# indygreg/python-zstandard

Hardware: AMD Instinct MI355X
Metric: GB/s uncompressed throughput, batch decompress of 128 KiB level-3 frames (the decompress half of BASELINE.json's metric; the compress half on the same inputs is this line's 'compress' object) (higher is better)
Workload: dtype u8

## Files before the change

### python-zstandard_amd/csrc/zhip_decode_pipeline.hpp

```cpp
#pragma once
#include "zhip_decode_kernel.hpp"

ZH_DEV void zp_pack_fse(ZdLDS& L, uint32_t* T, uint32_t llLog, uint32_t ofLog, uint32_t mlLog)
{
    const uint32_t lane = zh_lane();
    for (uint32_t u = lane; u < ZP_FSE_CELLS / 2; u += 64) {
        const uint32_t lg = u < 256 ? llLog : u < 512 ? mlLog : ofLog;
        const uint32_t local = (2 * u) & (u < 512 ? 511u : 255u);
        uint32_t pair = 0;
        for (uint32_t k = 0; k < 2; k++) {
            uint32_t cell = 0;
            if (local + k < (1u << lg)) {
                const uint32_t e = L.fse[2 * u + k];
                cell = ((e >> 19) << 10) | (((e & 1023) + (1u << lg)) >> ((e >> 10) & 15));
            }
            pair |= cell << (16 * k);
        }
        T[u] = pair;
    }
}

struct ZpHdr { uint32_t pos, blockMax, hasChecksum, skippable; uint64_t fcs; };
ZH_DEV int zp_frame_header(const ZhipPipeArgs& a, const uint8_t* src, uint32_t srcSize, ZpHdr& h)
{
// ... 934 lines not shown
            uint32_t r[ZP_FSE_CELLS / 128];
#pragma unroll
            for (uint32_t q = 0; q < ZP_FSE_CELLS / 128; q++) r[q] = src[lane + 64 * q];
#pragma unroll
            for (uint32_t q = 0; q < ZP_FSE_CELLS / 128; q++) dstw[lane + 64 * q] = r[q];
        }
        static_assert(ZQ_FRAMES <= 15, "the ring's last column is where the lanes without a frame write");
        uint32_t* const col = L.ring + (active ? slot : 15u);
        const bool idle = isSpare || !active;
        const uint16_t* const Tm = idle ? (const uint16_t*)&L.spare : (const uint16_t*)(L.tab + (size_t)slot * ZP_K2_STRIDE) + tabOff;
        ZdMeta* const m = a.meta + (active ? i : 0u);
        const uint32_t fi = active ? (MB ? a.itemFrame[i] : i) : 0u;
        const uint32_t f = a.first + fi;
        uint32_t nbSeq = 0, logs = 0;
        int32_t pos = 0, pb = -(1 << 30), fin = 0;
        const uint8_t* p0 = (const uint8_t*)a.counters;
        bool ok = active;
        ZpVec16 v0, v1; v0.a = v0.b = v0.c = v0.d = 0; v1 = v0;
        int32_t tb = 0;
        if (active) {
            const uint8_t* src = a.src + a.srcSegs[2 * (size_t)f];
            const uint8_t* p = src + m->seqOff; const uint8_t* end = src + m->seqEnd;
            const uint32_t size = (uint32_t)(end - p);
            logs = m->logs;
            const uint32_t lastB = size ? p[size - 1] : 0u;
            if (lastB == 0) ok = false;
            else {
                nbSeq = m->nbSeq;
                const uint32_t mis = (uint32_t)((uintptr_t)p & 15);
                p0 = p - mis; fin = (int32_t)(8 * mis);
                const int32_t topByte = (int32_t)(mis + size) - 1;
                tb = topByte & ~15;
                v0 = zq_fetch(p0, tb - 16 * (int32_t)role); v1 = zq_fetch(p0, tb - 16 * (int32_t)(role + 4));
                pb = tb - 128;
                pos = 8 * topByte + zh_highbit32(lastB);
            }
        }
        if (ok) { zq_commit(col, tb - 16 * (int32_t)role, v0); zq_commit(col, tb - 16 * (int32_t)(role + 4), v1); }
        zh_sync();
        const uint32_t llLog = logs & 255, ofLog = (logs >> 8) & 255, mlLog = (logs >> 16) & 255;
        const uint32_t myLog = idle ? 9u : role == 0 ? ofLog : role == 1 ? mlLog : llLog;
        const uint32_t kk = 31 - myLog, size = 1u << myLog;
        const uint16_t* const Tb = Tm - size;
        uint32_t state;
        {   const uint32_t initOff = role == 0 ? llLog : role == 1 ? llLog + ofLog : 0u;
            state = idle ? size : size + zq_field(col, pos - (int32_t)(initOff + myLog), myLog);
            pos -= (int32_t)(llLog + ofLog + mlLog); }
        const uint32_t nTrips = zh_first(zh_wave_max(nbSeq)) + 5;
        uint32_t rep0 = 1, rep1 = 4, rep2 = 8;
        if (a.dictEntropy) { rep0 = a.dictEntropy->rep[0]; rep1 = a.dictEntropy->rep[1]; rep2 = a.dictEntropy->rep[2]; }
        if (MB && active && a.frameRecs[fi].firstItem != i) { rep0 = ZP_SYM_REP(0); rep1 = ZP_SYM_REP(1); rep2 = ZP_SYM_REP(2); }
        uint32_t fin0 = rep0, fin1 = rep1, fin2 = rep2;
        rep0 = zh_opaque(rep0); rep1 = zh_opaque(rep1); rep2 = zh_opaque(rep2);
        ZpVec16* outp;
        {
            const uint32_t per = ((nTrips - 5 + 3) & ~3u) + 8;
            const uint32_t nAct = (uint32_t)zh_popc64(zh_ballot(active)) >> 2;
            const uint32_t need16 = per * nAct / 2;
            const uint32_t room16 = zh_first(zh_atomic_add(a.counters + 7, lane == 0 ? need16 : 0u));
            const uint32_t room = room16 * 2;
            if ((uint64_t)room16 + need16 + a.counters[8] > a.arenaBudget16) {
                if (active && isOF) { m->path = 2; if (!MB) { const uint32_t q = zh_atomic_add(a.fallbackCount, 1u); a.fallbackList[q] = f; } }
                zh_sync();
                continue;
            }
            const uint32_t start = room + slot * per + 4;
            if (active && isOF) a.bases[2 * (size_t)i] = start;
            outp = (ZpVec16*)(a.seqArena + (isOF && active ? (size_t)start - 4 : (size_t)room + per - 4));
        }
        const uint32_t outStep = isOF && active ? 2u : 0u;
        uint32_t g1lo = 0, g1hi = 0, g2lo = 0, g2hi = 0, g3lo = 0, g3hi = 0;
        ZpVec16 w0, w1; w0.a = w0.b = w0.c = w0.d = 0; w1 = w0;
        int32_t boff = tb - 16 * (int32_t)role, posEnd = pos; ZpVec16 blk = v0;
        uint32_t pe0 = 0, pe1 = 0, pqE = 0, pbits = 0, pbase = 1;
        for (uint32_t n0 = 0; n0 < nTrips; n0 += 4) {
            zh_sync();
            zq_commit_all(col, boff, blk);
            {   const int32_t t = pb + 128 - (((pos >> 5) << 2) + 4);
                boff = pb - 16 * (int32_t)role + ((int32_t)(role * 16) <= t ? 0 : 128);
                blk = zq_fetch(p0, boff);
                int32_t cnt = (t >> 4) + 1; cnt = cnt < 0 ? 0 : cnt > 4 ? 4 : cnt;
                pb -= 16 * cnt; }
#pragma unroll
            for (uint32_t u = 0; u < 4; u++) {
                const uint32_t n = n0 + u;
                const uint32_t cell = Tb[state];
                ZQ_F1();
                const uint32_t val = pbase + zh_bfe(zh_alignbit(pe1, pe0, pqE), 0, pbits);
                const uint32_t mlv = zh_quad<1>(val), llv = zh_quad<2>(val);
                const uint32_t idx = val - (llv < 1u ? llv : 1u);
                const uint32_t vm3 = val - 3;
                const uint32_t newOff = vm3 < ZP_OF_LIMIT ? vm3 : ZP_OF_LIMIT;
                const uint32_t c3 = val > 3 ? newOff : rep0 - 1;
                const bool i0 = idx == 0, i2 = idx == 2, le1 = idx <= 1;
                const uint32_t a01 = i0 ? rep0 : rep1, b23 = i2 ? rep2 : c3;
                const uint32_t offset = le1 ? a01 : b23;
                ZQ_F2();
                const uint32_t sym = cell >> 10, x = cell & 1023;
                const uint32_t inf = info[sym];
                const uint32_t nb = (uint32_t)__builtin_clz(x) - kk;
                ZQ_F2();
                rep2 = le1 ? rep2 : rep1; rep1 = i0 ? rep1 : rep0; rep0 = offset;
                if (MB) {
                    const bool wasLast = n == nbSeq;
                    fin0 = wasLast ? rep0 : fin0; fin1 = wasLast ? rep1 : fin1; fin2 = wasLast ? rep2 : fin2;
                }
                {   const uint32_t plo = llv | (mlv << 17), phi = (mlv >> 15) | (offset << 3);
                    if (u == 0) {
                        w0.a = g1lo; w0.b = g1hi; w0.c = g2lo; w0.d = g2hi; w1.a = g3lo; w1.b = g3hi; w1.c = plo; w1.d = phi;
#if defined(ZQ_DIAG_NOSTORE)
                        outp += outStep;
#elif defined(ZQ_NT_STORE)
                        {   typedef uint32_t zq_v4 __attribute__((ext_vector_type(4)));
                            zq_v4 t0 = { w0.a, w0.b, w0.c, w0.d }, t1 = { w1.a, w1.b, w1.c, w1.d };
                            __builtin_nontemporal_store(t0, (zq_v4*)outp); __builtin_nontemporal_store(t1, (zq_v4*)(outp + 1)); outp += outStep; }
#else
                        outp[0] = w0; outp[1] = w1; outp += outStep;
#endif
                    } else if (u == 1) { g1lo = plo; g1hi = phi; } else if (u == 2) { g2lo = plo; g2hi = phi; } else { g3lo = plo; g3hi = phi; } }
                ZQ_F2();
                const uint32_t bits = isOF ? sym : inf >> 24;
                const uint32_t P = zh_quad_add<0xCF>(zh_quad_add<0xD3>(bits, bits), bits);
                const uint32_t R = zh_quad_add<0xFE>(zh_quad_add<0xF9>(nb, nb), nb);
                const uint32_t totE = zh_quad<2>(P), totN = zh_quad<0>(R);
                const int32_t pE = pos - (int32_t)totE;
                const int32_t qS = pE - (int32_t)R, qE = pos - (int32_t)P;
                const uint32_t* const wS = (const uint32_t*)((const uint8_t*)col + (zh_bfe((uint32_t)qS, 5, 5) << 6));
                const uint32_t* const wE = (const uint32_t*)((const uint8_t*)col + (zh_bfe((uint32_t)qE, 5, 5) << 6));
                const uint32_t s0 = wS[0], s1 = wS[16];
                pe0 = wE[0]; pe1 = wE[16];
                ZQ_F2();
                pqE = (uint32_t)qE; pbits = bits;
                posEnd = n + 1 == nbSeq ? pE : posEnd;
                pos = pE - (int32_t)totN;
                pbase = isOF ? 1u << (sym & 31) : inf & 0xFFFFFFu;
                ZQ_F2();
                state = (x << nb) + zh_bfe(zh_alignbit(s1, s0, (uint32_t)qS), 0, nb);
                state = zh_pin(state);
            }
            ZH_KEEP4(w0.a, w0.b, w0.c, w0.d); ZH_KEEP4(w1.a, w1.b, w1.c, w1.d);
        }
        if (active && isOF) {
            const int err = !ok ? ZE_CORRUPTION : posEnd != fin ? ZE_CORRUPTION : 0;
            if (err) { m->status = err; m->path = 0; if (!MB) { a.status[f] = err; a.outSizes[f] = 0; } }
            if (MB) { uint32_t* r = a.itemReps + 4 * (size_t)i; r[0] = fin0; r[1] = fin1; r[2] = fin2; }
        }
        zh_sync();
    }
}

#ifndef ZP_ASM_BYTES
#define ZP_ASM_BYTES ZD_ASM_BYTES
#endif
struct ZpExecLDS {
    uint8_t asmb[ZP_ASM_BYTES + 64]; uint16_t mBeg[64]; uint16_t mEnd[64]; uint32_t misc[8];
#if defined(ZP_K3_DIAG_FLOOR) && defined(ZP_FLOOR_LDSPAD)
    uint8_t floorPad[ZP_FLOOR_LDSPAD];
#endif
    uint16_t uEnd[64], uLit[64], dstL[64], dstM[64], lenL[64], lenM[64]; uint32_t srcL[64], srcM[64];
};

ZH_DEV void zp_ld32_lds(const uint8_t* q, uint32_t len, uint64_t r[4])
{
    r[0] = zh_ld64(q); r[1] = zh_ld64(q + 8); r[2] = zh_ld64(q + 16);
    r[3] = zh_ld64(q + (len >= 8 ? len - 8 : 0u));
}

#ifndef ZP_LIT_SHORT
#define ZP_LIT_SHORT 16
#endif
#ifndef ZP_FAR_SHORT
#define ZP_FAR_SHORT 16
#endif
#ifndef ZP_K3_NT
#define ZP_K3_NT 0
#endif
#if ZP_K3_NT & 1
#define ZP_SEQ_LD(p) zh_ldq_nt(p)
#define ZP_LIT_LD64(p) zh_ld64_nt(p)
#else
#define ZP_SEQ_LD(p) (*(p))
#define ZP_LIT_LD64(p) zh_ld64(p)
#endif
#if ZP_K3_NT & 2
#define ZP_FAR_LD64(p) zh_ld64_nt(p)
#else
#define ZP_FAR_LD64(p) zh_ld64(p)
#endif
#define ZD_TP(P, i) do { if (PROF) ZD_T(P, i); } while (0)
ZH_DEV uint32_t zp_sym_resolve(uint32_t v, uint32_t R0, uint32_t R1, uint32_t R2)
{
    if (v <= ZP_OF_LIMIT) return v;
    if (v > ZP_SYM_TOP) return 0xFFFFFFFFu;
    const uint32_t k = (v - (ZP_OF_LIMIT + 1)) >> 23;
    const uint32_t d = ZP_SYM_REP(k) - v;
    const uint32_t r = k == 0 ? R0 : k == 1 ? R1 : R2;
    return r > d ? r - d : 0xFFFFFFFFu;
}

#define ZP_BSYNC() zh_sync()
#ifndef ZP_HIST_KEEP
#define ZP_HIST_KEEP ((ZP_ASM_BYTES * 5u / 16u) & ~15u)
#define ZP_HIST_SLIDE (2u * ZP_HIST_KEEP + 16u)
#endif
static_assert((ZP_HIST_SLIDE >= 2 * ZP_HIST_KEEP + 16 || ZP_HIST_KEEP == 0) && ZP_HIST_KEEP % 16 == 0 && ZP_HIST_SLIDE < ZP_ASM_BYTES, "the slide's source and destination must not overlap");
#ifndef ZP_K3_LITCOPIES
#define ZP_K3_LITCOPIES 3
#endif
enum { ZP_LM_ANY = 0, ZP_LM_ARENA = 1, ZP_LM_RAW = 2, ZP_LM_RLE = 3 };
template <bool DICT, bool PROF, bool MB, int LM>
ZH_DEVFN int zp_exec_block(const ZhipPipeArgs& a, ZpExecLDS& L, const ZdMeta& m, uint32_t t, const uint8_t* src, uint8_t* dst, uint32_t cap, uint64_t cap64,
                           uint32_t blockMax, uint32_t& opRef, uint32_t R0, uint32_t R1, uint32_t R2, ZdProf& P)
{
    const uint32_t lane = zh_lane();
    const uint64_t* seqs = a.seqArena + a.bases[2 * (size_t)t];
    const bool litRLE = LM == ZP_LM_ANY ? m.litMode == 2 : LM == ZP_LM_RLE;
    const bool litRaw = LM == ZP_LM_ANY ? m.litMode == 0 : LM == ZP_LM_RAW;
    const uint32_t rleByte = m.litOff;
    const uint8_t* litPtr = litRaw ? src + m.litOff : a.litArena + (size_t)a.bases[2 * (size_t)t + 1] * 16;
    const uint8_t* const dictEnd = DICT ? a.dictContent + a.dictContentSize : dst;
    const uint32_t dictSize = DICT ? a.dictContentSize : 0u;
    uint32_t hOff = 0;
    uint8_t* asmb = L.asmb;
    const uint32_t blockStart = MB ? opRef : 0u;
    uint32_t op = blockStart, lp = 0, done = 0;
    uint32_t carry = 0;
    const uint32_t nbSeq = m.nbSeq;
    uint64_t qNext = lane < nbSeq ? ZP_SEQ_LD(seqs + lane) : 0;
    const uint32_t lane0 = lane;
    while (done < nbSeq) {
        const uint32_t avail = nbSeq - done < 64 ? nbSeq - done : 64;
        uint32_t myLL = 0, myML = 0, myOF = 1;
        if (lane < avail) { const uint64_t q = qNext; myLL = ZP_SEQ_LL(q); myML = ZP_SEQ_ML(q); myOF = ZP_SEQ_OF(q); if (MB) myOF = zp_sym_resolve(myOF, R0, R1, R2); }
        if (MB && zh_ballot(lane < avail && myOF == ZP_OF_LIMIT)) return ZP_RC_FALLBACK;
        uint32_t incL = zh_scan_add(myLL), incT = zh_scan_add(myLL + myML);
        const uint64_t fits = zh_ballot(lane < avail && incT + carry <= ZP_ASM_BYTES - hOff);
        uint32_t cnt = (uint32_t)zh_popc64(fits);
        const bool big = cnt == 0;
        if (big) cnt = 1;
        qNext = done + cnt + lane < nbSeq ? ZP_SEQ_LD(seqs + done + cnt + lane) : 0;
        const bool act = lane < cnt;
        if (!act) { myLL = 0; myML = 0; myOF = 1; }
        const uint32_t totL = zh_bcast(incL, cnt - 1), totT = zh_bcast(incT, cnt - 1);
        if (lp + totL > m.litSize) return ZE_CORRUPTION;
        if ((uint64_t)op + totT > cap) return ZE_DST_TOO_SMALL;
        if (op + totT - blockStart > blockMax) return ZE_CORRUPTION;
        const uint32_t litStart = lp + incL - myLL;
        const uint32_t ob = op - carry;
        const uint32_t oRel = incT - (myLL + myML) + carry, mRel = oRel + myLL;
        if (zh_ballot(act && myOF - 1 >= ob + mRel + dictSize)) return ZE_CORRUPTION;
        if (big) {
            if (lane < carry) dst[ob + lane] = asmb[lane];
            carry = 0;
            zd_fence();
            const uint32_t bll = zh_bcast(myLL, 0), bml = zh_bcast(myML, 0), bof = zh_bcast(myOF, 0);
            if (litRLE) zd_fill_wave(dst + op, rleByte, bll); else zd_copy_wave(dst + op, litPtr + lp, bll);
            zd_fence();
            zd_match_wave(dst, dictEnd, op + bll, bof, bml);
            zd_fence();
            op += totT; lp += totL; done += 1;
            hOff = 0; asmb = L.asmb;
            continue;
        }
        ZD_TP(P, ZP_STAGE);
        const int32_t sAbs = (int32_t)(ob + mRel) - (int32_t)myOF;
        const bool hasM = act && myML > 0;
        const bool farM = hasM && sAbs + (int32_t)myML <= (int32_t)ob;
        uint32_t nearSkip = 0;
        {
            uint64_t rl[4], rm[4];
            const bool shortL = act && myLL > 0 && myLL <= ZP_LIT_SHORT;
            const bool arenaLit = !litRaw;
            if (arenaLit && !litRLE) {
                const uint8_t* q = litPtr + (shortL ? litStart : 0u);
                rl[0] = ZP_LIT_LD64(q); rl[3] = ZP_LIT_LD64(q + (shortL && myLL >= 8 ? myLL - 8 : 0u));
                if (ZP_LIT_SHORT > 16) { rl[1] = ZP_LIT_LD64(q + 8); rl[2] = ZP_LIT_LD64(q + 16); } else { rl[1] = 0; rl[2] = 0; }
            } else
            if (shortL && !litRLE) zd_ld32(litPtr + litStart, myLL, rl);
            const bool pre = hasM && !farM && sAbs < (int32_t)ob;
            const uint32_t preLen = pre ? (uint32_t)((int32_t)ob - sAbs) : 0u;
            nearSkip = preLen;
            const uint32_t lenMi = farM ? myML : preLen;
            const bool strad = DICT && (farM || pre) && sAbs < 0 && sAbs + (int32_t)lenMi > 0;
            const uint8_t* const mSrc = !DICT || sAbs >= 0 ? dst + sAbs : dictEnd + sAbs;
            const bool shortM = (farM || pre) && lenMi <= ZP_FAR_SHORT && !strad;
            const bool inH = (farM || pre) && sAbs >= (int32_t)(ob - hOff);
            if (!zh_ballot(shortM && !inH && sAbs >= 0 && (uint64_t)sAbs + 32 > cap64) && cap64 >= 32) {
                const uint8_t* q = shortM && !inH ? mSrc : dst;
                rm[0] = ZP_FAR_LD64(q); rm[3] = ZP_FAR_LD64(q + (shortM && lenMi >= 8 ? lenMi - 8 : 0u));
                if (ZP_FAR_SHORT > 16) { rm[1] = ZP_FAR_LD64(q + 8); rm[2] = ZP_FAR_LD64(q + 16); } else { rm[1] = 0; rm[2] = 0; }
            } else
            if (shortM && !inH) zd_ld32(mSrc, lenMi, rm);
            if (shortM && inH) { const uint8_t* hq = asmb + (sAbs - (int32_t)ob); rm[0] = zh_ld64(hq); rm[1] = 0; rm[2] = 0; rm[3] = zh_ld64(hq + (lenMi >= 8 ? lenMi - 8 : 0u)); }
            const bool longL = act && myLL > ZP_LIT_SHORT && !litRLE, longM = (farM || pre) && !shortM && !strad;
            const uint32_t uL = longL ? (myLL + 15) >> 4 : 0u, uM = longM ? (lenMi + 15) >> 4 : 0u;
            const uint32_t ue = zh_scan_add(uL + uM);
            const uint32_t U = zh_bcast(ue, 63);
            zh_v16 uv; uv.lo = 0; uv.hi = 0; uint8_t* udp = asmb;
            if (U) {
                L.uEnd[lane] = (uint16_t)ue; L.uLit[lane] = (uint16_t)uL;
                L.srcL[lane] = litStart; L.dstL[lane] = (uint16_t)oRel; L.lenL[lane] = (uint16_t)myLL;
                L.srcM[lane] = (uint32_t)sAbs; L.dstM[lane] = (uint16_t)mRel; L.lenM[lane] = (uint16_t)lenMi;
                ZP_BSYNC();
#define ZP_UNIT(u) do { uint32_t j_ = 0; for (uint32_t stp_ = 32; stp_; stp_ >>= 1) if (L.uEnd[j_ + stp_ - 1] <= (u)) j_ += stp_; \
                    uint32_t k_ = (u) - (j_ ? (uint32_t)L.uEnd[j_ - 1] : 0u); const uint32_t nl_ = L.uLit[j_]; const bool isL_ = k_ < nl_; if (!isL_) k_ -= nl_; \
                    const uint32_t len_ = isL_ ? L.lenL[j_] : L.lenM[j_]; const uint32_t off_ = 16 * k_ + 16 <= len_ ? 16 * k_ : len_ - 16; \
                    const int32_t sm_ = (int32_t)L.srcM[j_]; \
                    if (!isL_ && sm_ >= (int32_t)(ob - hOff)) { const uint8_t* h_ = asmb + (sm_ - (int32_t)ob) + off_; uv.lo = zh_ld64(h_); uv.hi = zh_ld64(h_ + 8); } \
                    else uv = zh_ld128(isL_ ? litPtr + L.srcL[j_] + off_ : (!DICT || sm_ >= 0 ? dst + sm_ : dictEnd + sm_) + off_); \
                    udp = asmb + (isL_ ? L.dstL[j_] : L.dstM[j_]) + off_; } while (0)
                if (lane < U) ZP_UNIT(lane);
            }
            if (litRLE) { for (int k = 0; k < 4; k++) rl[k] = 0x0101010101010101ull * rleByte; }
            if (shortL) zd_st32(asmb + oRel, myLL, rl);
            if (shortM) zd_st32(asmb + mRel, lenMi, rm);
            if (DICT) for (uint64_t mk = zh_ballot(strad); mk; mk &= mk - 1) {
                const uint32_t l = (uint32_t)zh_ctz64(mk);
                const uint32_t d = zh_shfl(mRel, l), nn = zh_shfl(lenMi, l);
                const int32_t s0 = (int32_t)zh_shfl((uint32_t)sAbs, l);
                for (uint32_t j = lane; j < nn; j += 64) asmb[d + j] = (uint8_t)zd_hist_byte(dst, dictEnd, s0 + (int32_t)j);
            }
            if (U) {
                if (lane < U) { zh_st64(udp, uv.lo); zh_st64(udp + 8, uv.hi); }
                for (uint32_t u = lane + 64; u < U; u += 64) { ZP_UNIT(u); zh_st64(udp, uv.lo); zh_st64(udp + 8, uv.hi); }
#undef ZP_UNIT
            }
        }
        if (litRLE) {
            for (uint64_t mk = zh_ballot(act && myLL > ZP_LIT_SHORT); mk; mk &= mk - 1) {
                const uint32_t l = (uint32_t)zh_ctz64(mk);
                const uint32_t d = zh_shfl(oRel, l), n = zh_shfl(myLL, l);
                for (uint32_t j = lane; j < n; j += 64) asmb[d + j] = (uint8_t)rleByte;
            }
        }
        L.mBeg[lane] = (uint16_t)(act ? mRel : 0xFFFF); L.mEnd[lane] = (uint16_t)(act ? mRel + myML : 0xFFFF);
        ZP_BSYNC();
        ZD_TP(P, ZP_EXEC1);
        bool pending = hasM && !farM;
        uint64_t need = 0;
        if (pending) {
            const uint32_t a0 = sAbs > (int32_t)ob ? (uint32_t)(sAbs - (int32_t)ob) : 0;
            uint32_t b0 = (uint32_t)(sAbs + (int32_t)myML - (int32_t)ob);
            if (b0 > mRel) b0 = mRel;
            uint32_t lo = 0, hi = 0;
            for (uint32_t stp = 32; stp; stp >>= 1) { if (lo + stp <= 64 && L.mEnd[lo + stp - 1] <= a0) lo += stp; }
            for (uint32_t stp = 32; stp; stp >>= 1) { if (hi + stp <= 64 && L.mBeg[hi + stp - 1] < b0) hi += stp; }
            if (hi > lane) hi = lane;
            if (lo < hi) need = (hi >= 64 ? ~0ull : ((1ull << hi) - 1)) & ~((1ull << lo) - 1);
        }
        const uint64_t nearMask = zh_ballot(pending);
        need &= nearMask;
        uint64_t doneMask = ~nearMask;
        for (;;) {
            const uint64_t pend = zh_ballot(pending);
            if (!pend) break;
            const uint64_t longReady = zh_ballot(pending && myML > ZD_COOP_LEN && (need & ~doneMask) == 0);
            {
                const bool ready = pending && myML <= ZD_COOP_LEN && (need & ~doneMask) == 0;
                if (ready) {
                    const uint32_t nLen = myML - nearSkip, nSrc = (uint32_t)(sAbs + (int32_t)nearSkip - (int32_t)ob), nDst = mRel + nearSkip;
                    if (myOF >= nLen) {
                        uint64_t rr[4];
                        zp_ld32_lds(asmb + nSrc, nLen, rr);
                        zd_st32(asmb + nDst, nLen, rr);
                    } else {
                        uint32_t done = 0, span = myOF;
                        while (done < nLen) {
                            uint32_t c = span; if (c > nLen - done) c = nLen - done; if (c > 32) c = 32;
                            uint64_t rr[4];
                            zp_ld32_lds(asmb + nDst + done - span, c, rr);
                            zd_st32(asmb + nDst + done, c, rr);
                            done += c;
                            if (c == span) span += span;
                        }
                    }
                    pending = false;
                }
                uint64_t newDone = zh_ballot(ready);
                for (uint64_t lm = longReady; lm; lm &= lm - 1) {
                    const uint32_t pf = (uint32_t)zh_ctz64(lm);
                    const uint32_t Frel = zh_shfl(mRel, pf), fml = zh_shfl(myML, pf), fof = zh_shfl(myOF, pf);
                    const int32_t fs = (int32_t)(ob + Frel) - (int32_t)fof;
                    if (fof >= 64) {
                        for (uint32_t c = 0; c < fml; c += 64) {
                            const uint32_t j = c + lane;
                            if (j < fml) { const int32_t sp = fs + (int32_t)j; asmb[Frel + j] = sp >= (int32_t)(ob - hOff) ? asmb[sp - (int32_t)ob] : (DICT ? (uint8_t)zd_hist_byte(dst, dictEnd, sp) : dst[sp]); }
                            if (fof < fml) ZP_BSYNC();
                        }
                    } else {
                        uint32_t idx = lane % fof; const uint32_t adv = 64 % fof;
                        for (uint32_t j = lane; j < fml; j += 64) {
                            const int32_t sp = fs + (int32_t)idx;
                            asmb[Frel + j] = sp >= (int32_t)(ob - hOff) ? asmb[sp - (int32_t)ob] : (DICT ? (uint8_t)zd_hist_byte(dst, dictEnd, sp) : dst[sp]);
                            idx += adv; if (idx >= fof) idx -= fof;
                        }
                    }
                    if (lane == pf) pending = false;
                    newDone |= 1ull << pf;
                    if (lm & (lm - 1)) ZP_BSYNC();
                }
                doneMask |= newDone;
            }
            ZP_BSYNC();
        }
        ZD_TP(P, ZP_EXEC2);
        qNext = zh_opaque64(qNext);
        const uint32_t totB = totT + carry, whole = totB & ~15u;
        {
            uint8_t* out = dst + ob;
            const uint32_t j0 = lane * 16;
            if (j0 < whole) { const zh_v16 v = *(const zh_v16*)(asmb + j0); *(zh_v16*)(out + j0) = v; }
            if (whole > 1024) for (uint32_t j = j0 + 1024; j < whole; j += 1024) { const zh_v16 v = *(const zh_v16*)(asmb + zh_opaque(j)); *(zh_v16*)(out + j) = v; }
        }
        carry = totB - whole;
        hOff += whole;
        ZP_BSYNC();
        if (hOff > ZP_HIST_SLIDE) {
            const uint32_t s0 = hOff - ZP_HIST_KEEP, n = ZP_HIST_KEEP + carry;
            for (uint32_t j = lane * 16; j < n; j += 1024) { const zh_v16 v = *(const zh_v16*)(L.asmb + s0 + j); *(zh_v16*)(L.asmb + j) = v; }
            hOff = ZP_HIST_KEEP;
            ZP_BSYNC();
        }
        asmb = L.asmb + hOff;
        ZD_TP(P, ZP_FLUSH);
        op += totT; lp += totL; done += cnt;
    }
    if (lane < carry) dst[op - carry + lane] = asmb[lane];
    zd_fence();
    const uint32_t rest = m.litSize - lp;
    if ((uint64_t)op + rest > cap) return ZE_DST_TOO_SMALL;
    if (op + rest - blockStart > blockMax) return ZE_CORRUPTION;
    if (litRLE) zd_fill_wave(dst + op, rleByte, rest); else zd_copy_wave(dst + op, litPtr + lp, rest);
    op += rest;
    opRef = op;
    return 0;
}

template <bool DICT, bool PROF, bool MB>
ZH_DEVFN int zp_exec_block_by_mode(const ZhipPipeArgs& a, ZpExecLDS& L, const ZdMeta& m, uint32_t t, const uint8_t* src, uint8_t* dst, uint32_t cap, uint64_t cap64,
                                   uint32_t blockMax, uint32_t& opRef, uint32_t R0, uint32_t R1, uint32_t R2, ZdProf& P)
{
    constexpr int copies = DICT ? 1 : ZP_K3_LITCOPIES;
#define ZP_XB(LM_) zp_exec_block<DICT, PROF, MB, LM_>(a, L, m, t, src, dst, cap, cap64, blockMax, opRef, R0, R1, R2, P)
    if constexpr (copies >= 2) { if (m.litMode != 0 && m.litMode != 2) return ZP_XB(ZP_LM_ARENA); }
    if constexpr (copies >= 3) { if (m.litMode == 0) return ZP_XB(ZP_LM_RAW); return ZP_XB(ZP_LM_RLE); }
    else return ZP_XB(ZP_LM_ANY);
#undef ZP_XB
}


ZH_DEVFN int zp_exec_frame_end(ZpExecLDS& L, const uint8_t* dst, uint32_t op, uint32_t fcsLo, uint32_t fcsHi, uint32_t hasChecksum, uint32_t checksum, uint32_t ckLater)
{
    const uint32_t lane = zh_lane();
    const uint64_t fcs = (uint64_t)fcsLo | ((uint64_t)fcsHi << 32);
    if (fcs != ~0ull && fcs != op) return ZE_CORRUPTION;
    if ((hasChecksum & 1) && !ckLater) {
        zd_fence();
        zh_sync();
        if (zh_opaque(lane) == 0) L.misc[0] = (uint32_t)ze_xxh64(dst, op);
        zh_sync();
        const uint32_t digest = zh_first(L.misc[0]);
        zh_sync();
        if (digest != checksum) return ZE_CHECKSUM_WRONG;
    }
    return 0;
}

#ifdef ZP_K3_DIAG_FLOOR
#include "../../tests/ubench/k3_floor_diag.hpp"
#endif
template <bool DICT, bool PROF>
ZH_DEVFN int zp_exec_frame(const ZhipPipeArgs& a, ZpExecLDS& L, uint32_t i, uint32_t* pProduced, ZdProf& P)
{
    const ZdMeta m = a.meta[i];
    const uint32_t f = a.first + i;
    const uint8_t* src = a.src + a.srcSegs[2 * (size_t)f];
    uint8_t* dst = a.dst + a.dstSegs[2 * (size_t)f];
    const uint64_t cap64 = a.dstSegs[2 * (size_t)f + 1];
    const uint32_t cap = cap64 > 0x7FFFFFFFull ? 0x7FFFFFFFu : (uint32_t)cap64;
    uint32_t op = 0;
#ifdef ZP_K3_DIAG_FLOOR
    int e = zp_exec_block_floor<DICT, PROF, false>(a, L, m, i, src, dst, cap, cap64, m.blockMax, op);
#else
    int e = zp_exec_block_by_mode<DICT, PROF, false>(a, L, m, i, src, dst, cap, cap64, m.blockMax, op, 1, 4, 8, P);
#endif
    if (e) return e;
    e = zp_exec_frame_end(L, dst, op, m.fcsLo, m.fcsHi, m.hasChecksum, m.checksum, a.ckLater);
    if (e) return e;
    *pProduced = op;
    return 0;
}

template <bool DICT>
ZH_DEVFN int zp_exec_frame_mb(const ZhipPipeArgs& a, ZpExecLDS& L, uint32_t i, uint32_t* pProduced, ZdProf& P)
{
    const ZpFrameRec rec = a.frameRecs[i];
    const uint32_t f = a.first + i;
    const uint8_t* src = a.src + a.srcSegs[2 * (size_t)f];
    uint8_t* dst = a.dst + a.dstSegs[2 * (size_t)f];
    const uint64_t cap64 = a.dstSegs[2 * (size_t)f + 1];
    const uint32_t cap = cap64 > 0x7FFFFFFFull ? 0x7FFFFFFFu : (uint32_t)cap64;
    uint32_t R0 = 1, R1 = 4, R2 = 8;
    if (a.dictEntropy) { R0 = a.dictEntropy->rep[0]; R1 = a.dictEntropy->rep[1]; R2 = a.dictEntropy->rep[2]; }
    uint32_t op = 0;
    for (uint32_t bi = 0; bi < rec.nItems; bi++) {
        const uint32_t t = rec.firstItem + bi;
        const ZdMeta m = a.meta[t];
        if (m.path == 0) return m.status ? m.status : ZE_CORRUPTION;
        if (m.path == 2) return ZP_RC_FALLBACK;
        if (m.path >= 3) {
            const uint32_t size = m.litSize;
            if ((uint64_t)op + size > cap) return ZE_DST_TOO_SMALL;
            if (m.path == 3) zd_copy_wave(dst + op, src + m.litOff, size); else zd_fill_wave(dst + op, m.litOff, size);
            zd_fence();
            op += size;
            continue;
        }
        const int e = zp_exec_block_by_mode<DICT, false, true>(a, L, m, t, src, dst, cap, cap64, rec.blockMax, op, R0, R1, R2, P);
        if (e) return e;
        zd_fence();
        if (m.nbSeq) {
            const uint32_t* r = a.itemReps + 4 * (size_t)t;
            const uint32_t n0 = zp_sym_resolve(r[0], R0, R1, R2), n1 = zp_sym_resolve(r[1], R0, R1, R2), n2 = zp_sym_resolve(r[2], R0, R1, R2);
            R0 = n0; R1 = n1; R2 = n2;
        }
    }
    const int e = zp_exec_frame_end(L, dst, op, rec.fcsLo, rec.fcsHi, rec.hasChecksum, rec.checksum, a.ckLater);
    if (e) return e;
    *pProduced = op;
    return 0;
}

template <bool DICT, bool PROF, bool MB = false>
ZH_DEVFN void zp_exec_body(const ZhipPipeArgs& a, ZpExecLDS& L)
{
    const uint32_t lane = zh_lane();
    for (;;) {
        const uint32_t got = zh_atomic_add(a.counters + 2, lane == 0 ? 1u : 0u);
        if (zh_opaque(lane) == 0) L.misc[7] = got;
        zh_sync();
        const uint32_t k = zh_first(L.misc[7]);
        zh_sync();
        if (k >= a.count) break;
        const uint32_t i = k;
        if (MB) { if (a.frameRecs[i].path != 1) continue; }
        else {
        if (a.meta[i].path != 1) continue;
        }
        uint32_t produced = 0;
        ZdProf P; P.on = PROF && a.prof != nullptr;
        if (PROF && P.on) { for (int q = 0; q < ZP_N; q++) P.acc[q] = 0; P.t0 = zd_clock(); }
        int err;
        if constexpr (MB) err = zp_exec_frame_mb<DICT>(a, L, i, &produced, P);
        else err = zp_exec_frame<DICT, PROF>(a, L, i, &produced, P);
        if (PROF && P.on) { ZD_T(P, ZP_RAW); if (lane == 0) for (int q = 0; q < ZP_N; q++) if (P.acc[q]) zh_atomic_add64(a.prof + 16 + q, P.acc[q]); }
        zh_sync();
        if (zh_opaque(lane) == 0) {
            if (MB && err == ZP_RC_FALLBACK) { const uint32_t q = zh_atomic_add(a.fallbackCount, 1u); a.fallbackList[q] = a.first + i;
                                               a.status[a.first + i] = ZE_CORRUPTION; a.outSizes[a.first + i] = 0; }
            else { a.status[a.first + i] = err; a.outSizes[a.first + i] = err ? 0 : produced; }
        }
    }
}

ZH_DEVFN void zp_check_body(const ZhipPipeArgs& a)
{
    if (a.counters[12] == 0) return;
    const uint32_t lane = zh_lane();
    for (uint32_t i = zh_block() * 64 + lane; i < a.count; i += zh_nblocks() * 64) {
        uint32_t has, want, path;
        if (a.itemCap) { const ZpFrameRec& r = a.frameRecs[i]; has = r.hasChecksum & 1u; want = r.checksum; path = r.path; }
        else { const ZdMeta& m = a.meta[i]; has = m.hasChecksum & 1u; want = m.checksum; path = m.path; }
        if (!has || path == 2) continue;
        const uint32_t f = a.first + i;
        if (a.status[f] != 0) continue;
        const uint8_t* dst = a.dst + a.dstSegs[2 * (size_t)f];
        const uint64_t n = a.outSizes[f];
        if ((uint32_t)ze_xxh64(dst, (uint32_t)n) != want) { a.status[f] = ZE_CHECKSUM_WRONG; a.outSizes[f] = 0; }
    }
}
```

### python-zstandard_amd/csrc/zhip_device.hpp

```cpp
#pragma once
#include <stdint.h>
#include <stddef.h>

#ifndef ZHIP_EMU
#include <hip/hip_runtime.h>
#define ZH_DEV __device__ __forceinline__
#ifdef ZD_NOINLINE
#define ZH_DEVFN __device__ __attribute__((noinline))
#else
#define ZH_DEVFN __device__
#endif
#define ZH_COLD __device__ __attribute__((noinline))
#define ZH_GLOBAL extern "C" __global__
#define ZH_SHARED __shared__
#define ZH_CONST __device__ const
#define ZH_LDS_CPTR(type, p) ((const __attribute__((address_space(3))) type*)(p))

ZH_DEV uint32_t zh_lane() { return threadIdx.x; }
ZH_DEV uint32_t zh_block() { return blockIdx.x; }
ZH_DEV uint32_t zh_nblocks() { return gridDim.x; }
ZH_DEV void zh_sync() { __syncthreads(); }
ZH_DEV void zh_wave_fence() { __builtin_amdgcn_fence(__ATOMIC_RELEASE, "wavefront"); __builtin_amdgcn_wave_barrier(); __builtin_amdgcn_fence(__ATOMIC_ACQUIRE, "wavefront"); }
ZH_DEV uint64_t zh_ballot(bool p) { return __ballot(p); }
ZH_DEV uint32_t zh_shfl(uint32_t v, uint32_t srcLane) { return (uint32_t)__shfl((int)v, (int)srcLane, 64); }
ZH_DEV uint32_t zh_shfl_up(uint32_t v, uint32_t d) { return (uint32_t)__shfl_up((int)v, d, 64); }
ZH_DEV uint32_t zh_first(uint32_t v) { return (uint32_t)__builtin_amdgcn_readfirstlane((int)v); }
ZH_DEV uint32_t zh_bcast(uint32_t v, uint32_t l) { return (uint32_t)__builtin_amdgcn_readlane((int)v, (int)l); }
template <int K> ZH_DEV uint32_t zh_quad(uint32_t v) { return (uint32_t)__builtin_amdgcn_mov_dpp((int)v, K * 0x55, 0xf, 0xf, false); }
template <int CTRL> ZH_DEV uint32_t zh_quad_add(uint32_t acc, uint32_t v) { return acc + (uint32_t)__builtin_amdgcn_mov_dpp((int)v, CTRL, 0xf, 0xf, false); }
ZH_DEV uint32_t zh_atomic_inc(uint32_t* p) { return atomicAdd(p, 1u); }
ZH_DEV uint32_t zh_atomic_add(uint32_t* p, uint32_t v) { return atomicAdd(p, v); }
ZH_DEV void zh_atomic_add64(unsigned long long* p, unsigned long long v) { atomicAdd(p, v); }
ZH_DEV void zh_atomic_max(uint32_t* p, uint32_t v) { atomicMax(p, v); }
ZH_DEV void zh_atomic_or(uint32_t* p, uint32_t v) { atomicOr(p, v); }
ZH_DEV void zh_lds_atomic_or(uint32_t* p, uint32_t v) { atomicOr(p, v); }
ZH_DEV void zh_lds_atomic_inc(uint32_t* p) { atomicAdd(p, 1u); }
ZH_DEV uint32_t zh_lds_atomic_add(uint32_t* p, uint32_t v) { return atomicAdd(p, v); }
ZH_DEV void zh_lds_atomic_max(uint32_t* p, uint32_t v) { atomicMax(p, v); }
ZH_DEV uint32_t zh_wave_max(uint32_t v) { for (int d = 32; d; d >>= 1) { uint32_t o = (uint32_t)__shfl_xor((int)v, d, 64); v = o > v ? o : v; } return v; }
ZH_DEV void ze_fence() { __builtin_amdgcn_fence(__ATOMIC_SEQ_CST, "workgroup"); }
ZH_DEV uint32_t zh_opaque(uint32_t v) { asm volatile("" : "+v"(v)); return v; }
ZH_DEV uint64_t zh_opaque64(uint64_t v) { asm volatile("" : "+v"(v)); return v; }
ZH_DEV int zh_popc64(uint64_t v) { return __popcll(v); }
ZH_DEV int zh_ctz64(uint64_t v) { return __ffsll((unsigned long long)v) - 1; }
ZH_DEV int zh_clz64(uint64_t v) { return __clzll((long long)v); }
ZH_DEV int zh_highbit32(uint32_t v) { return 31 - __clz((int)v); }
#define ZH_SCHED_FENCE() __builtin_amdgcn_sched_barrier(0)
#define ZH_KEEP4(a, b, c, d) asm volatile("" :: "v"(a), "v"(b), "v"(c), "v"(d))
ZH_DEV uint32_t zh_bfe(uint32_t v, uint32_t off, uint32_t width) { return __builtin_amdgcn_ubfe(v, off, width); }
ZH_DEV uint32_t zh_alignbit(uint32_t hi, uint32_t lo, uint32_t sh) { return __builtin_amdgcn_alignbit(hi, lo, sh); }

#else
#include "zhip_device_emu.hpp"
#endif

#ifndef ZHIP_EMU
ZH_DEV uint32_t zh_pin(uint32_t v) { asm("" : "+v"(v)); return v; }
#else
ZH_DEV uint32_t zh_pin(uint32_t v) { return v; }
#endif
typedef uint64_t __attribute__((aligned(1))) zh_u64u;
typedef uint32_t __attribute__((aligned(1))) zh_u32u;
typedef uint16_t __attribute__((aligned(1))) zh_u16u;
struct __attribute__((packed, aligned(1))) zh_v16 { uint64_t lo, hi; };
ZH_DEV zh_v16 zh_ld128(const uint8_t* p) { return *(const zh_v16*)p; }
ZH_DEV uint64_t zh_ld64(const uint8_t* p) { return *(const zh_u64u*)p; }
ZH_DEV uint32_t zh_ld32(const uint8_t* p) { return *(const zh_u32u*)p; }
ZH_DEV uint32_t zh_ld16(const uint8_t* p) { return *(const zh_u16u*)p; }
ZH_DEV uint32_t zh_ld24(const uint8_t* p) { return (uint32_t)p[0] | ((uint32_t)p[1] << 8) | ((uint32_t)p[2] << 16); }
ZH_DEV void zh_st64(uint8_t* p, uint64_t v) { *(zh_u64u*)p = v; }
ZH_DEV void zh_st32(uint8_t* p, uint32_t v) { *(zh_u32u*)p = v; }
ZH_DEV void zh_st16(uint8_t* p, uint16_t v) { *(zh_u16u*)p = v; }
ZH_DEV uint64_t zh_lt_mask() { return (1ull << zh_lane()) - 1; }
#ifndef ZHIP_EMU
typedef uint32_t __attribute__((ext_vector_type(4))) zh_v4raw;
typedef zh_v4raw __attribute__((aligned(1))) zh_v4rawu;
ZH_DEV uint64_t zh_ld64_nt(const uint8_t* p) { return __builtin_nontemporal_load((const zh_u64u*)p); }
ZH_DEV zh_v16 zh_ld128_nt(const uint8_t* p) { const zh_v4raw v = __builtin_nontemporal_load((const zh_v4rawu*)p); zh_v16 r; r.lo = (uint64_t)v.x | ((uint64_t)v.y << 32); r.hi = (uint64_t)v.z | ((uint64_t)v.w << 32); return r; }
ZH_DEV uint64_t zh_ldq_nt(const uint64_t* p) { return __builtin_nontemporal_load(p); }
#else
ZH_DEV uint64_t zh_ld64_nt(const uint8_t* p) { return zh_ld64(p); }
ZH_DEV zh_v16 zh_ld128_nt(const uint8_t* p) { return zh_ld128(p); }
ZH_DEV uint64_t zh_ldq_nt(const uint64_t* p) { return *p; }
#endif

#ifndef ZHIP_EMU
ZH_DEV uint32_t zh_scan_add(uint32_t v)
{
    v += (uint32_t)__builtin_amdgcn_update_dpp(0, (int)v, 0x111, 0xf, 0xf, false);
    v += (uint32_t)__builtin_amdgcn_update_dpp(0, (int)v, 0x112, 0xf, 0xf, false);
    v += (uint32_t)__builtin_amdgcn_update_dpp(0, (int)v, 0x114, 0xf, 0xf, false);
    v += (uint32_t)__builtin_amdgcn_update_dpp(0, (int)v, 0x118, 0xf, 0xf, false);
    v += (uint32_t)__builtin_amdgcn_update_dpp(0, (int)v, 0x142, 0xa, 0xf, false);
    v += (uint32_t)__builtin_amdgcn_update_dpp(0, (int)v, 0x143, 0xc, 0xf, false);
    return v;
}
#endif
```

Before: 404.9.

## Pack per-item unit descriptors into one LDS record and use scalar base pointers

The per-lane unit bookkeeping that sat in eight separate LDS arrays is packed into a single 16-byte record per lane. An optional owner table lets each lane find its starting item with a ballot and clz instead of a binary search. Base pointers for dst, the sequence arena and the literal arena are made wave-uniform so global loads can use a scalar base with 32-bit offsets. Together these aim to cut LDS traffic, address arithmetic and VGPR use in the execute stage, at the cost of bit-packing limits that rest on static_asserts and more macro complexity.

```diff
diff --git a/python-zstandard_amd/csrc/zhip_decode_pipeline.hpp b/python-zstandard_amd/csrc/zhip_decode_pipeline.hpp
--- a/python-zstandard_amd/csrc/zhip_decode_pipeline.hpp
+++ b/python-zstandard_amd/csrc/zhip_decode_pipeline.hpp
@@ -1110,13 +1110,38 @@
 #ifndef ZP_ASM_BYTES
 #define ZP_ASM_BYTES ZD_ASM_BYTES
 #endif
+#ifndef ZP_K3_UNITREC
+#define ZP_K3_UNITREC 1
+#endif
+#ifndef ZP_K3_UNITOWN
+#define ZP_K3_UNITOWN 1
+#endif
+#if !ZP_K3_UNITREC
+#undef ZP_K3_UNITOWN
+#define ZP_K3_UNITOWN 0
+#endif
+struct alignas(16) ZpUnitRec { uint32_t w[4]; };
+static_assert(ZP_ASM_BYTES < (1u << 13), "ZpUnitRec: lengths up to and positions below ZP_ASM_BYTES in 13 bits");
+static_assert(ZF_BLOCK_MAX <= (1u << 17), "ZpUnitRec: a long literal run starts below 2^17");
+static_assert((ZP_ASM_BYTES + 15u * 128u) / 16u < (1u << 10), "ZpUnitRec: an item's first unit in 10 bits");
+static_assert((ZP_ASM_BYTES + 15u) / 16u < (1u << 9), "ZpUnitRec: an item's literal units in 9 bits");
 struct ZpExecLDS {
     uint8_t asmb[ZP_ASM_BYTES + 64]; uint16_t mBeg[64]; uint16_t mEnd[64]; uint32_t misc[8];
 #if defined(ZP_K3_DIAG_FLOOR) && defined(ZP_FLOOR_LDSPAD)
     uint8_t floorPad[ZP_FLOOR_LDSPAD];
 #endif
+#if ZP_K3_UNITREC
+    ZpUnitRec rec[64]; uint16_t uEnd[64];
+#if ZP_K3_UNITOWN
+    uint8_t own[64];
+#endif
+#else
     uint16_t uEnd[64], uLit[64], dstL[64], dstM[64], lenL[64], lenM[64]; uint32_t srcL[64], srcM[64];
+#endif
 };
+#if ZP_K3_UNITREC
+static_assert(sizeof(ZpExecLDS) <= ZP_ASM_BYTES + 1632, "K3's waves per CU rest on this size (5 728 bytes at ZP_ASM_BYTES = 4 096)");
+#endif
 
 ZH_DEV void zp_ld32_lds(const uint8_t* q, uint32_t len, uint64_t r[4])
 {
@@ -1165,17 +1190,38 @@
 #ifndef ZP_K3_LITCOPIES
 #define ZP_K3_LITCOPIES 3
 #endif
+#ifndef ZP_K3_SBASE
+#define ZP_K3_SBASE 1
+#endif
 enum { ZP_LM_ANY = 0, ZP_LM_ARENA = 1, ZP_LM_RAW = 2, ZP_LM_RLE = 3 };
+ZH_DEV void zp_ld32_at(const uint8_t* base, uint32_t off, uint32_t len, uint64_t r[4])
+{
+    const bool ge8 = len >= 8;
+    const uint32_t o2 = len & 4, o1 = o2 + (len & 2);
+    uint64_t a0 = 0, a1 = 0, a2 = 0, a3 = 0; uint32_t b4 = 0, b2 = 0, b1 = 0;
+    if (ge8) a0 = zh_ld64(base + off);
+    if (len > 16) a1 = zh_ld64(base + (off + 8));
+    if (len > 24) a2 = zh_ld64(base + (off + 16));
+    if (ge8) a3 = zh_ld64(base + (off + len - 8));
+    if (!ge8 && (len & 4)) b4 = zh_ld32(base + off);
+    if (!ge8 && (len & 2)) b2 = zh_ld16(base + (off + o2));
+    if (!ge8 && (len & 1)) b1 = base[off + o1];
+    r[0] = a0; r[1] = a1; r[2] = a2;
+    r[3] = ge8 ? a3 : (uint64_t)b4 | ((uint64_t)b2 << (8 * o2)) | ((uint64_t)b1 << (8 * o1));
+}
 template <bool DICT, bool PROF, bool MB, int LM>
 ZH_DEVFN int zp_exec_block(const ZhipPipeArgs& a, ZpExecLDS& L, const ZdMeta& m, uint32_t t, const uint8_t* src, uint8_t* dst, uint32_t cap, uint64_t cap64,
                            uint32_t blockMax, uint32_t& opRef, uint32_t R0, uint32_t R1, uint32_t R2, ZdProf& P)
 {
     const uint32_t lane = zh_lane();
+    constexpr bool SB = ZP_K3_SBASE && !DICT;
+    if (SB) dst = zh_uniform_ptr(dst);
     const uint64_t* seqs = a.seqArena + a.bases[2 * (size_t)t];
     const bool litRLE = LM == ZP_LM_ANY ? m.litMode == 2 : LM == ZP_LM_RLE;
     const bool litRaw = LM == ZP_LM_ANY ? m.litMode == 0 : LM == ZP_LM_RAW;
     const uint32_t rleByte = m.litOff;
     const uint8_t* litPtr = litRaw ? src + m.litOff : a.litArena + (size_t)a.bases[2 * (size_t)t + 1] * 16;
+    if (SB) { seqs = zh_uniform_ptr(seqs); litPtr = zh_uniform_ptr(litPtr); }
     const uint8_t* const dictEnd = DICT ? a.dictContent + a.dictContentSize : dst;
     const uint32_t dictSize = DICT ? a.dictContentSize : 0u;
     uint32_t hOff = 0;
@@ -1184,7 +1230,8 @@
     uint32_t op = blockStart, lp = 0, done = 0;
     uint32_t carry = 0;
     const uint32_t nbSeq = m.nbSeq;
-    uint64_t qNext = lane < nbSeq ? ZP_SEQ_LD(seqs + lane) : 0;
+#define ZP_SEQ_AT(first) (SB ? ZP_SEQ_LD((const uint64_t*)((const uint8_t*)seqs + ((first) + lane) * 8u)) : ZP_SEQ_LD(seqs + (first) + lane))
+    uint64_t qNext = lane < nbSeq ? ZP_SEQ_AT(0u) : 0;
     const uint32_t lane0 = lane;
     while (done < nbSeq) {
         const uint32_t avail = nbSeq - done < 64 ? nbSeq - done : 64;
@@ -1196,7 +1243,7 @@
         uint32_t cnt = (uint32_t)zh_popc64(fits);
         const bool big = cnt == 0;
         if (big) cnt = 1;
-        qNext = done + cnt + lane < nbSeq ? ZP_SEQ_LD(seqs + done + cnt + lane) : 0;
+        qNext = done + cnt + lane < nbSeq ? ZP_SEQ_AT(done + cnt) : 0;
         const bool act = lane < cnt;
         if (!act) { myLL = 0; myML = 0; myOF = 1; }
         const uint32_t totL = zh_bcast(incL, cnt - 1), totT = zh_bcast(incT, cnt - 1);
@@ -1230,11 +1277,17 @@
             const bool shortL = act && myLL > 0 && myLL <= ZP_LIT_SHORT;
             const bool arenaLit = !litRaw;
             if (arenaLit && !litRLE) {
+                if (SB) {
+                    const uint32_t q = shortL ? litStart : 0u;
+                    rl[0] = ZP_LIT_LD64(litPtr + q); rl[3] = ZP_LIT_LD64(litPtr + (q + (shortL && myLL >= 8 ? myLL - 8 : 0u)));
+                    if (ZP_LIT_SHORT > 16) { rl[1] = ZP_LIT_LD64(litPtr + (q + 8)); rl[2] = ZP_LIT_LD64(litPtr + (q + 16)); } else { rl[1] = 0; rl[2] = 0; }
+                } else {
                 const uint8_t* q = litPtr + (shortL ? litStart : 0u);
                 rl[0] = ZP_LIT_LD64(q); rl[3] = ZP_LIT_LD64(q + (shortL && myLL >= 8 ? myLL - 8 : 0u));
                 if (ZP_LIT_SHORT > 16) { rl[1] = ZP_LIT_LD64(q + 8); rl[2] = ZP_LIT_LD64(q + 16); } else { rl[1] = 0; rl[2] = 0; }
+                }
             } else
-            if (shortL && !litRLE) zd_ld32(litPtr + litStart, myLL, rl);
+            if (shortL && !litRLE) { if (SB) zp_ld32_at(litPtr, litStart, myLL, rl); else zd_ld32(litPtr + litStart, myLL, rl); }
             const bool pre = hasM && !farM && sAbs < (int32_t)ob;
             const uint32_t preLen = pre ? (uint32_t)((int32_t)ob - sAbs) : 0u;
             nearSkip = preLen;
@@ -1243,19 +1296,57 @@
             const uint8_t* const mSrc = !DICT || sAbs >= 0 ? dst + sAbs : dictEnd + sAbs;
             const bool shortM = (farM || pre) && lenMi <= ZP_FAR_SHORT && !strad;
             const bool inH = (farM || pre) && sAbs >= (int32_t)(ob - hOff);
-            if (!zh_ballot(shortM && !inH && sAbs >= 0 && (uint64_t)sAbs + 32 > cap64) && cap64 >= 32) {
+            const bool slack = SB ? !zh_ballot(shortM && !inH && (uint32_t)sAbs + 32 > cap) && cap >= 32
+                                  : !zh_ballot(shortM && !inH && sAbs >= 0 && (uint64_t)sAbs + 32 > cap64) && cap64 >= 32;
+            if (slack && SB) {
+                const uint32_t q = shortM && !inH ? (uint32_t)sAbs : 0u;
+                rm[0] = ZP_FAR_LD64(dst + q); rm[3] = ZP_FAR_LD64(dst + (q + (shortM && lenMi >= 8 ? lenMi - 8 : 0u)));
+                if (ZP_FAR_SHORT > 16) { rm[1] = ZP_FAR_LD64(dst + (q + 8)); rm[2] = ZP_FAR_LD64(dst + (q + 16)); } else { rm[1] = 0; rm[2] = 0; }
+            } else
+            if (slack) {
                 const uint8_t* q = shortM && !inH ? mSrc : dst;
                 rm[0] = ZP_FAR_LD64(q); rm[3] = ZP_FAR_LD64(q + (shortM && lenMi >= 8 ? lenMi - 8 : 0u));
                 if (ZP_FAR_SHORT > 16) { rm[1] = ZP_FAR_LD64(q + 8); rm[2] = ZP_FAR_LD64(q + 16); } else { rm[1] = 0; rm[2] = 0; }
             } else
-            if (shortM && !inH) zd_ld32(mSrc, lenMi, rm);
+            if (shortM && !inH) { if (SB) zp_ld32_at(dst, (uint32_t)sAbs, lenMi, rm); else zd_ld32(mSrc, lenMi, rm); }
             if (shortM && inH) { const uint8_t* hq = asmb + (sAbs - (int32_t)ob); rm[0] = zh_ld64(hq); rm[1] = 0; rm[2] = 0; rm[3] = zh_ld64(hq + (lenMi >= 8 ? lenMi - 8 : 0u)); }
             const bool longL = act && myLL > ZP_LIT_SHORT && !litRLE, longM = (farM || pre) && !shortM && !strad;
             const uint32_t uL = longL ? (myLL + 15) >> 4 : 0u, uM = longM ? (lenMi + 15) >> 4 : 0u;
             const uint32_t ue = zh_scan_add(uL + uM);
             const uint32_t U = zh_bcast(ue, 63);
             zh_v16 uv; uv.lo = 0; uv.hi = 0; uint8_t* udp = asmb;
+#define ZP_UNIT_GLOBAL(isL_, lo_, sm_, off_) uv = zh_ld128((isL_) ? litPtr + (lo_) : (!DICT || (sm_) >= 0 ? dst + (sm_) : dictEnd + (sm_)) + (off_))
             if (U) {
+#if ZP_K3_UNITREC
+                ZpUnitRec mine;
+                mine.w[0] = (uint32_t)sAbs; mine.w[1] = litStart | (oRel << 17); mine.w[2] = myLL | (lenMi << 13); mine.w[3] = mRel | ((ue - (uL + uM)) << 13) | (uL << 23);
+                L.rec[lane] = mine;
+#if ZP_K3_UNITOWN
+                L.own[lane] = 0xFF;
+                zh_wave_fence();
+                const uint32_t first = ue - (uL + uM);
+                if (uL + uM && first < 64) L.own[first] = (uint8_t)lane;
+                if (U > 64) L.uEnd[lane] = (uint16_t)ue;
+                ZP_BSYNC();
+                const uint64_t starts = zh_ballot(L.own[lane] != 0xFF);
+#define ZP_UNIT_J0(j_) j_ = L.own[63 - zh_clz64(starts & (~0ull >> (63 - lane)))]
+#else
+                L.uEnd[lane] = (uint16_t)ue;
+                ZP_BSYNC();
+#define ZP_UNIT_J0(j_) ZP_UNIT_J(lane, j_)
+#endif
+#define ZP_UNIT_J(u, j_) for (uint32_t stp_ = 32; stp_; stp_ >>= 1) if (L.uEnd[j_ + stp_ - 1] <= (u)) j_ += stp_
+#define ZP_UNIT0() do { uint32_t j_ = 0; ZP_UNIT_J0(j_); ZP_UNIT_DO(lane, j_); } while (0)
+#define ZP_UNIT(u) do { uint32_t j_ = 0; ZP_UNIT_J(u, j_); ZP_UNIT_DO(u, j_); } while (0)
+#define ZP_UNIT_DO(u, j_) do { \
+                    const ZpUnitRec r_ = L.rec[j_]; \
+                    uint32_t k_ = (u) - ((r_.w[3] >> 13) & 0x3FFu); const uint32_t nl_ = r_.w[3] >> 23; const bool isL_ = k_ < nl_; if (!isL_) k_ -= nl_; \
+                    const uint32_t len_ = (isL_ ? r_.w[2] : r_.w[2] >> 13) & 0x1FFFu; const uint32_t off_ = 16 * k_ + 16 <= len_ ? 16 * k_ : len_ - 16; \
+                    const int32_t sm_ = (int32_t)r_.w[0]; \
+                    if (!isL_ && sm_ >= (int32_t)(ob - hOff)) { const uint8_t* h_ = asmb + (sm_ - (int32_t)ob) + off_; uv.lo = zh_ld64(h_); uv.hi = zh_ld64(h_ + 8); } \
+                    else ZP_UNIT_GLOBAL(isL_, (r_.w[1] & 0x1FFFFu) + off_, sm_, off_); \
+                    udp = asmb + ((isL_ ? r_.w[1] >> 17 : r_.w[3]) & 0x1FFFu) + off_; } while (0)
+#else
                 L.uEnd[lane] = (uint16_t)ue; L.uLit[lane] = (uint16_t)uL;
                 L.srcL[lane] = litStart; L.dstL[lane] = (uint16_t)oRel; L.lenL[lane] = (uint16_t)myLL;
                 L.srcM[lane] = (uint32_t)sAbs; L.dstM[lane] = (uint16_t)mRel; L.lenM[lane] = (uint16_t)lenMi;
@@ -1265,9 +1356,11 @@
                     const uint32_t len_ = isL_ ? L.lenL[j_] : L.lenM[j_]; const uint32_t off_ = 16 * k_ + 16 <= len_ ? 16 * k_ : len_ - 16; \
                     const int32_t sm_ = (int32_t)L.srcM[j_]; \
                     if (!isL_ && sm_ >= (int32_t)(ob - hOff)) { const uint8_t* h_ = asmb + (sm_ - (int32_t)ob) + off_; uv.lo = zh_ld64(h_); uv.hi = zh_ld64(h_ + 8); } \
-                    else uv = zh_ld128(isL_ ? litPtr + L.srcL[j_] + off_ : (!DICT || sm_ >= 0 ? dst + sm_ : dictEnd + sm_) + off_); \
+                    else ZP_UNIT_GLOBAL(isL_, L.srcL[j_] + off_, sm_, off_); \
                     udp = asmb + (isL_ ? L.dstL[j_] : L.dstM[j_]) + off_; } while (0)
-                if (lane < U) ZP_UNIT(lane);
+#define ZP_UNIT0() ZP_UNIT(lane)
+#endif
+                if (lane < U) ZP_UNIT0();
             }
             if (litRLE) { for (int k = 0; k < 4; k++) rl[k] = 0x0101010101010101ull * rleByte; }
             if (shortL) zd_st32(asmb + oRel, myLL, rl);
@@ -1282,6 +1375,11 @@
                 if (lane < U) { zh_st64(udp, uv.lo); zh_st64(udp + 8, uv.hi); }
                 for (uint32_t u = lane + 64; u < U; u += 64) { ZP_UNIT(u); zh_st64(udp, uv.lo); zh_st64(udp + 8, uv.hi); }
 #undef ZP_UNIT
+#undef ZP_UNIT0
+#undef ZP_UNIT_J
+#undef ZP_UNIT_J0
+#undef ZP_UNIT_DO
+#undef ZP_UNIT_GLOBAL
             }
         }
         if (litRLE) {
@@ -1342,14 +1440,14 @@
                     if (fof >= 64) {
                         for (uint32_t c = 0; c < fml; c += 64) {
                             const uint32_t j = c + lane;
-                            if (j < fml) { const int32_t sp = fs + (int32_t)j; asmb[Frel + j] = sp >= (int32_t)(ob - hOff) ? asmb[sp - (int32_t)ob] : (DICT ? (uint8_t)zd_hist_byte(dst, dictEnd, sp) : dst[sp]); }
+                            if (j < fml) { const int32_t sp = fs + (int32_t)j; asmb[Frel + j] = sp >= (int32_t)(ob - hOff) ? asmb[sp - (int32_t)ob] : (DICT ? (uint8_t)zd_hist_byte(dst, dictEnd, sp) : SB ? dst[(uint32_t)sp] : dst[sp]); }
                             if (fof < fml) ZP_BSYNC();
                         }
                     } else {
                         uint32_t idx = lane % fof; const uint32_t adv = 64 % fof;
                         for (uint32_t j = lane; j < fml; j += 64) {
                             const int32_t sp = fs + (int32_t)idx;
-                            asmb[Frel + j] = sp >= (int32_t)(ob - hOff) ? asmb[sp - (int32_t)ob] : (DICT ? (uint8_t)zd_hist_byte(dst, dictEnd, sp) : dst[sp]);
+                            asmb[Frel + j] = sp >= (int32_t)(ob - hOff) ? asmb[sp - (int32_t)ob] : (DICT ? (uint8_t)zd_hist_byte(dst, dictEnd, sp) : SB ? dst[(uint32_t)sp] : dst[sp]);
                             idx += adv; if (idx >= fof) idx -= fof;
                         }
                     }
@@ -1365,10 +1463,10 @@
         qNext = zh_opaque64(qNext);
         const uint32_t totB = totT + carry, whole = totB & ~15u;
         {
-            uint8_t* out = dst + ob;
-            const uint32_t j0 = lane * 16;
-            if (j0 < whole) { const zh_v16 v = *(const zh_v16*)(asmb + j0); *(zh_v16*)(out + j0) = v; }
-            if (whole > 1024) for (uint32_t j = j0 + 1024; j < whole; j += 1024) { const zh_v16 v = *(const zh_v16*)(asmb + zh_opaque(j)); *(zh_v16*)(out + j) = v; }
+            uint8_t* out = SB ? dst : dst + ob;
+            const uint32_t j0 = lane * 16, o0 = SB ? ob : 0u;
+            if (j0 < whole) { const zh_v16 v = *(const zh_v16*)(asmb + j0); *(zh_v16*)(out + (o0 + j0)) = v; }
+            if (whole > 1024) for (uint32_t j = j0 + 1024; j < whole; j += 1024) { const zh_v16 v = *(const zh_v16*)(asmb + zh_opaque(j)); *(zh_v16*)(out + (o0 + j)) = v; }
         }
         carry = totB - whole;
         hOff += whole;
@@ -1392,6 +1490,7 @@
     op += rest;
     opRef = op;
     return 0;
+#undef ZP_SEQ_AT
 }
 
 template <bool DICT, bool PROF, bool MB>
diff --git a/python-zstandard_amd/csrc/zhip_device.hpp b/python-zstandard_amd/csrc/zhip_device.hpp
--- a/python-zstandard_amd/csrc/zhip_device.hpp
+++ b/python-zstandard_amd/csrc/zhip_device.hpp
@@ -59,6 +59,16 @@
 #else
 ZH_DEV uint32_t zh_pin(uint32_t v) { return v; }
 #endif
+#ifndef ZHIP_EMU
+template <class T> ZH_DEV T* zh_uniform_ptr(T* p)
+{
+    const uint64_t v = (uint64_t)p;
+    const uint64_t u = (uint64_t)zh_first((uint32_t)v) | ((uint64_t)zh_first((uint32_t)(v >> 32)) << 32);
+    return (T*)(__attribute__((address_space(1))) T*)u;
+}
+#else
+template <class T> ZH_DEV T* zh_uniform_ptr(T* p) { return p; }
+#endif
 typedef uint64_t __attribute__((aligned(1))) zh_u64u;
 typedef uint32_t __attribute__((aligned(1))) zh_u32u;
 typedef uint16_t __attribute__((aligned(1))) zh_u16u;
```

Result: faster. 409.0, median of 6 (+1.0%).
